# avi22bhattacharya/ThinkDiff-mlre

Measured on NVIDIA B200. Metric: aligner_train_tokens_per_sec, higher is better.
Workload: dtype bf16

## Files before the change

thinkdiff_mlre_b200/csrc/gemm_host.cuh:

```cuda
#pragma once
#include <cstdio>
#include <cstring>
#include <atomic>
#include <mutex>
#include <vector>

#include "gemm_sm100.cuh"

namespace td {

inline char* last_error_buf() {
  static thread_local char buf[512] = "";
  return buf;
}
#define TD_FAIL(code, ...)                                        \
  do {                                                            \
    snprintf(td::last_error_buf(), 512, __VA_ARGS__);             \
    return (code);                                                \
  } while (0)
#define TD_CUDA(expr)                                                                             \
  do {                                                                                            \
    cudaError_t _e = (expr);                                                                      \
    if (_e != cudaSuccess) TD_FAIL(-100 - int(_e), "%s failed: %s", #expr, cudaGetErrorString(_e)); \
  } while (0)
// ... 140 lines not shown
                            bool mn_major, int box_rows) {
  if (!mn_major)
    return encode_2d(map, CU_TENSOR_MAP_DATA_TYPE_BFLOAT16, ptr, (cuuint64_t)K, (cuuint64_t)rows, (cuuint64_t)ld * 2, kBlockK,
                     (cuuint32_t)box_rows, CU_TENSOR_MAP_SWIZZLE_128B, CU_TENSOR_MAP_L2_PROMOTION_L2_256B);
  return encode_2d(map, CU_TENSOR_MAP_DATA_TYPE_BFLOAT16, ptr, (cuuint64_t)rows, (cuuint64_t)K, (cuuint64_t)ld * 2, 64, kBlockK,
                   CU_TENSOR_MAP_SWIZZLE_128B, CU_TENSOR_MAP_L2_PROMOTION_L2_256B);
}
inline int make_epilogue_map(CUtensorMap* map, const void* ptr, long long rows, long long cols, long long ld, bool f32) {
  if (f32)
    return encode_2d(map, CU_TENSOR_MAP_DATA_TYPE_FLOAT32, ptr, (cuuint64_t)cols, (cuuint64_t)rows, (cuuint64_t)ld * 4, 32, 32,
                     CU_TENSOR_MAP_SWIZZLE_128B, CU_TENSOR_MAP_L2_PROMOTION_NONE);
  return encode_2d(map, CU_TENSOR_MAP_DATA_TYPE_BFLOAT16, ptr, (cuuint64_t)cols, (cuuint64_t)rows, (cuuint64_t)ld * 2, 32, 32,
                   CU_TENSOR_MAP_SWIZZLE_64B, CU_TENSOR_MAP_L2_PROMOTION_NONE);
}

struct GemmOperand {
  const void* ptr;
  long long ld;
  bool mn_major;
};

inline size_t gemm_sk_workspace_bytes() { return sizeof(float) * (size_t)device_sm_count() * kSkSlotFloats; }

inline void plan_schedule(GemmParams& p, int max_workers, bool stream_k) {
  const int tiles = p.num_m_blocks * p.num_n_blocks;
  const int KB = p.num_k_blocks;
  int W = max_workers;
  if (tiles < W) {
    long long by_k = (long long)tiles * KB / kMinTailKBlocks;
    long long w = stream_k ? (by_k > tiles ? by_k : tiles) : tiles;
    W = int(w < max_workers ? w : max_workers);
    if (W < 1) W = 1;
  }
  p.workers = W;
  p.full_waves = tiles / W;
  const int R = tiles - p.full_waves * W;
  p.tail_workers = 0; p.tail_q = 0; p.tail_r = 0;
  if (stream_k && R > 0) {
    const long long units = (long long)R * KB;
    long long wt = units / kMinTailKBlocks;
    if (wt < R) wt = R;
    if (wt > W) wt = W;
    p.tail_workers = int(wt);
    p.tail_q = int(units / wt);
    p.tail_r = int(units % wt);
  }
}

template <int CTAS, bool A_MN, bool B_MN, int EPI>
int launch_gemm(GemmOperand a, GemmOperand b, GemmParams p, void* ws, cudaStream_t stream, const char* tag = "gemm") {
  using S = GemmSmem<CTAS, EPI>;
  if (p.M <= 0 || p.N <= 0) return TD_OK;
  if (p.N % 32) TD_FAIL(TD_ERR_UNSUPPORTED, "GEMM N=%d must be a multiple of 32", p.N);
  if (p.K <= 0) TD_FAIL(TD_ERR_ARG, "GEMM K=%d must be positive (caller zero-fills empty contractions)", p.K);
  CUtensorMap ma, mb, mo0, mo1, maux;
  ScatterMaps smaps;
  memset(&mo0, 0, sizeof(mo0)); memset(&mo1, 0, sizeof(mo1)); memset(&maux, 0, sizeof(maux)); memset(&smaps, 0, sizeof(smaps));
  int rc = make_operand_map(&ma, a.ptr, p.M, p.K, a.ld, A_MN, kBlockM);
  if (rc) return rc;
  rc = make_operand_map(&mb, b.ptr, p.N, p.K, b.ld, B_MN, kBlockN / CTAS);
  if (rc) return rc;
  if (EPI != EPI_F32_SCATTER && p.out0 != nullptr) {
    rc = make_epilogue_map(&mo0, p.out0, p.M, p.N, p.ld_out, EPI == EPI_F32);
    if (rc) return rc;
  }
  if (EPI == EPI_BIAS_GELU) {
    rc = make_epilogue_map(&mo1, p.out1, p.M, p.N, p.ld_out, false);
    if (rc) return rc;
// ... 17 lines not shown
  p.sk_partials = static_cast<float*>(ws);
  p.sched_counter = next_sched_counter();
  if (!p.sched_counter) TD_FAIL(TD_ERR_DRIVER, "cannot allocate the tile-scheduler counters");
  p.sk_flags = nullptr;
  if (p.tail_workers > 0) {
    p.sk_flags = next_sk_flags();
    if (!p.sk_flags) TD_FAIL(TD_ERR_DRIVER, "cannot allocate the stream-K flag pool");
  }

  auto kern = gemm_bf16_kernel<CTAS, A_MN, B_MN, EPI>;
  static std::atomic<bool> attr_set[kMaxDevices];
  const int dev = current_device();
  if (dev < 0 || dev >= kMaxDevices) TD_FAIL(TD_ERR_DRIVER, "no current CUDA device");
  if (!attr_set[dev].load(std::memory_order_acquire)) {
    TD_CUDA(cudaFuncSetAttribute(kern, cudaFuncAttributeMaxDynamicSharedMemorySize, S::kTotal));
    attr_set[dev].store(true, std::memory_order_release);
  }
  cudaLaunchConfig_t cfg;
  memset(&cfg, 0, sizeof(cfg));
  cfg.gridDim = dim3(p.workers * CTAS);
  cfg.blockDim = dim3(kGemmThreads);
  cfg.dynamicSmemBytes = S::kTotal;
  cfg.stream = stream;
  cudaLaunchAttribute attr[1];
  attr[0].id = cudaLaunchAttributeClusterDimension;
  attr[0].val.clusterDim.x = CTAS;
  attr[0].val.clusterDim.y = 1;
  attr[0].val.clusterDim.z = 1;
  cfg.attrs = attr;
  cfg.numAttrs = 1;
  ProfScope prof(tag, 2.0 * double(p.M) * double(p.N) * double(p.K), stream);
  TD_CUDA(cudaLaunchKernelEx(&cfg, kern, ma, mb, mo0, mo1, maux, smaps, p));
  return TD_OK;
}

}
```

thinkdiff_mlre_b200/csrc/gemm_sm100.cuh:

```cuda
#pragma once
#include "ptx_sm100.cuh"

namespace td {

enum EpiKind : int {
  EPI_BF16 = 0,
  EPI_BIAS_GELU = 1,
  EPI_BIAS_SSQ = 2,
  EPI_DGELU = 3,
  EPI_F32 = 4,
  EPI_F32_SCATTER = 5,
};
constexpr int kMaxPeers = 8;

struct GemmParams {
  int M, N, K;
  int num_m_blocks, num_n_blocks, num_k_blocks;
  int workers;
  int full_waves;
  int tail_workers;
  int tail_q, tail_r;
  float* sk_partials;
  int* sk_flags;
  int* sched_counter;
// ... 11 lines not shown
  int scatter_rows;
  int raster_group_m;
  int raster_rot_m;
  int* post_signal[kMaxPeers];
  int post_signal_n;
};
struct ScatterMaps {
  CUtensorMap m[kMaxPeers];
};

constexpr int kBlockM = 128;
constexpr int kBlockN = 256;
constexpr int kBlockK = 64;
constexpr int kUmmaK = 16;
constexpr int kGemmThreads = 320;
#ifndef TD_ROLES_HI
#define TD_ROLES_HI 1
#endif
constexpr int kEpiWarp0 = TD_ROLES_HI ? 0 : 2;
constexpr int kProducerWarp = TD_ROLES_HI ? 8 : 0;
constexpr int kMmaWarp = TD_ROLES_HI ? 9 : 1;
constexpr int kAccStages = 2;
constexpr int kMinTailKBlocks = 8;

constexpr int kEpiWarps = 8;
constexpr int kEpiColsPerWarp = kBlockN / (kEpiWarps / 4);
constexpr int kEpiChunks = kEpiColsPerWarp / 32;
constexpr int kSkSlotFloats = kEpiWarps * kEpiChunks * 32 * 32;

#ifndef TD_MAX_STAGES
#define TD_MAX_STAGES 7
#endif

template <int EPI> struct EpiStage { static constexpr int kBytesPerWarp = 4096; };
template <> struct EpiStage<EPI_DGELU> { static constexpr int kBytesPerWarp = 6144; };
template <> struct EpiStage<EPI_F32> { static constexpr int kBytesPerWarp = 8192; };
template <> struct EpiStage<EPI_F32_SCATTER> { static constexpr int kBytesPerWarp = 8192; };

template <int EPI> struct StageCap { static constexpr int kMax = TD_MAX_STAGES; };
#ifndef TD_NO_CORESIDENCY
template <> struct StageCap<EPI_BIAS_GELU> { static constexpr int kMax = 5; };
template <> struct StageCap<EPI_F32> { static constexpr int kMax = 5; };
template <> struct StageCap<EPI_F32_SCATTER> { static constexpr int kMax = 5; };
#endif

template <int CTAS, int EPI>
// ... 348 lines not shown
    if constexpr (EPI == EPI_DGELU) tma_prefetch_desc(&tmap_aux);
    for (int s = 0; s < kStages; ++s) {
      mbar_init(&full_bar[s], 1);
      mbar_init(&empty_bar[s], 1);
    }
    for (int s = 0; s < kAccStages; ++s) {
      mbar_init(&acc_full_bar[s], 1);
      mbar_init(&acc_empty_bar[s], kEpiWarps * CTAS);
    }
    for (int s = 0; s < 2 * kEpiWarps; ++s) mbar_init(&aux_bar[s], 1);
    for (int s = 0; s < kSchedStages; ++s) {
      mbar_init(&sched_full_bar[s], 1);
      mbar_init(&sched_empty_bar[s], kSchedConsumers);
    }
    fence_mbar_init();
  }
  if (warp == kMmaWarp) {
    tmem_alloc<CTAS>(tmem_slot, 512);
    tmem_relinquish<CTAS>();
  }
  tc_fence_before();
  if constexpr (CTAS == 2) cluster_sync_all(); else __syncthreads();
  tc_fence_after();
  const uint32_t tmem_base = *tmem_slot;
  const int num_workers = gridDim.x / CTAS;
  const int n_units = num_units(p);

  auto sched_consume = [&](int ss, uint32_t sphase, bool whole_warp) -> int {
    mbar_wait_cluster(&sched_full_bar[ss], sphase);
    const int unit = *reinterpret_cast<volatile int*>(&sched_unit[ss]);
    if (whole_warp) __syncwarp();
    if (!whole_warp || lane == 0) {
      if constexpr (CTAS == 1) mbar_arrive(&sched_empty_bar[ss]);
      else mbar_arrive_cluster(&sched_empty_bar[ss], 0);
    }
    return unit;
  };

  if (warp == kProducerWarp) {
    if (lane == 0) {
      int stage = 0, ss = 0;
      uint32_t phase = 0, sphase = 0;
      int claimed = leader ? atomicAdd(p.sched_counter, 1) : 0;
      while (true) {
        int unit;
        if (leader) {
// ... 27 lines not shown
              if constexpr (CTAS == 1) tma_load_2d(sa, &tmap_a, &full_bar[stage], k0, a_row0);
              else tma_load_2d_pair(sa, &tmap_a, &full_bar[stage], k0, a_row0);
            } else {
#pragma unroll
              for (int j = 0; j < kBlockM / 64; ++j) {
                if constexpr (CTAS == 1) tma_load_2d(sa + j * (kBlockK * 128), &tmap_a, &full_bar[stage], a_row0 + j * 64, k0);
                else tma_load_2d_pair(sa + j * (kBlockK * 128), &tmap_a, &full_bar[stage], a_row0 + j * 64, k0);
              }
            }
            if constexpr (!B_MN) {
              if constexpr (CTAS == 1) tma_load_2d(sb, &tmap_b, &full_bar[stage], k0, b_row0);
              else tma_load_2d_pair(sb, &tmap_b, &full_bar[stage], k0, b_row0);
            } else {
#pragma unroll
              for (int j = 0; j < kBRows / 64; ++j) {
                if constexpr (CTAS == 1) tma_load_2d(sb + j * (kBlockK * 128), &tmap_b, &full_bar[stage], b_row0 + j * 64, k0);
                else tma_load_2d_pair(sb + j * (kBlockK * 128), &tmap_b, &full_bar[stage], b_row0 + j * 64, k0);
              }
            }
            if (++stage == kStages) { stage = 0; phase ^= 1; }
          }
        });
      }
      if (leader) {
        __threadfence();
        if (atomicAdd(p.sched_counter + 1, 1) == num_workers - 1) {
          p.sched_counter[0] = 0;
          p.sched_counter[1] = 0;
          __threadfence();
        }
      }
    }
    __syncwarp();
  } else if (warp == kMmaWarp) {
    if (leader && lane == 0) {
      constexpr uint32_t idesc = make_idesc_bf16(kBlockM * CTAS, kBlockN, A_MN, B_MN);
      constexpr uint32_t a_lbo = A_MN ? kBlockK * 128 : 16, b_lbo = B_MN ? kBlockK * 128 : 16;
      constexpr uint32_t sbo = 1024;
      constexpr uint32_t a_kstep = A_MN ? kUmmaK * 128 : kUmmaK * 2;
      constexpr uint32_t b_kstep = B_MN ? kUmmaK * 128 : kUmmaK * 2;
      int stage = 0, acc = 0, ss = 0;
      uint32_t phase = 0, acc_phase = 0, sphase = 0;
      while (true) {
        const int unit = sched_consume(ss, sphase, false);
        if (++ss == kSchedStages) { ss = 0; sphase ^= 1; }
        if (unit < 0) break;
// ... 81 lines not shown
```

thinkdiff_mlre_b200/csrc/ptx_sm100.cuh:

```cuda
#pragma once
#include <cuda.h>
#include <cuda_bf16.h>
#include <cuda_runtime.h>
#include <stdint.h>

namespace td {

__device__ __forceinline__ uint32_t smem_u32(const void* p) {
  return static_cast<uint32_t>(__cvta_generic_to_shared(p));
}

__device__ __forceinline__ uint64_t global_timer_ns() {
  uint64_t t;
  asm volatile("mov.u64 %0, %%globaltimer;" : "=l"(t));
  return t;
}

__device__ __forceinline__ void mbar_init(uint64_t* bar, uint32_t count) {
  asm volatile("mbarrier.init.shared::cta.b64 [%0], %1;" ::"r"(smem_u32(bar)), "r"(count));
}
__device__ __forceinline__ void fence_mbar_init() {
  asm volatile("fence.mbarrier_init.release.cluster;" ::: "memory");
}
__device__ __forceinline__ void fence_proxy_async_smem() {
// ... 78 lines not shown
  int v;
  asm volatile("ld.acquire.gpu.global.s32 %0, [%1];" : "=r"(v) : "l"(p) : "memory");
  return v;
}
__device__ __forceinline__ int ld_relaxed_gpu(const int* p) {
  int v;
  asm volatile("ld.relaxed.gpu.global.s32 %0, [%1];" : "=r"(v) : "l"(p) : "memory");
  return v;
}
__device__ __forceinline__ void spin_until_set(const int* p) {
  if (ld_relaxed_gpu(p) == 0) {
    const uint64_t t0 = global_timer_ns();
    while (ld_relaxed_gpu(p) == 0) {
      __nanosleep(64);
      if (global_timer_ns() - t0 > TD_MBAR_TIMEOUT_NS) {
        printf("td: stream-K flag timeout block %d thread %d\n", blockIdx.x, threadIdx.x);
        __trap();
      }
    }
  }
  asm volatile("fence.acq_rel.gpu;" ::: "memory");
}

__device__ __forceinline__ uint32_t cluster_ctarank() {
  uint32_t r;
  asm volatile("mov.u32 %0, %%cluster_ctarank;" : "=r"(r));
  return r;
}
__device__ __forceinline__ void cluster_sync_all() {
  asm volatile("barrier.cluster.arrive.release.aligned;\n barrier.cluster.wait.acquire.aligned;" ::: "memory");
}

__device__ __forceinline__ void fence_tensormap_acquire(const CUtensorMap* m) {
  asm volatile("fence.proxy.tensormap::generic.acquire.sys [%0], 128;" ::"l"(m) : "memory");
}

__device__ __forceinline__ void tma_prefetch_desc(const CUtensorMap* m) {
  asm volatile("prefetch.tensormap [%0];" ::"l"(m) : "memory");
}
__device__ __forceinline__ void tma_load_2d(void* dst, const CUtensorMap* map, uint64_t* bar, int c0, int c1) {
  asm volatile(
      "cp.async.bulk.tensor.2d.shared::cluster.global.mbarrier::complete_tx::bytes [%0], [%1, {%3, %4}], [%2];" ::"r"(
          smem_u32(dst)),
      "l"(map), "r"(smem_u32(bar)), "r"(c0), "r"(c1)
      : "memory");
}
// ... 162 lines not shown
```

thinkdiff_mlre_b200/csrc/rowops_sm100.cuh:

```cuda
#pragma once
#include "ptx_sm100.cuh"

namespace td {

__device__ __forceinline__ uint4 ld_stream(const uint4* p) {
  uint4 r;
  asm("ld.global.nc.L1::no_allocate.v4.u32 {%0, %1, %2, %3}, [%4];"
      : "=r"(r.x), "=r"(r.y), "=r"(r.z), "=r"(r.w)
      : "l"(p));
  return r;
}
#ifndef TD_ST_VARIANT
#define TD_ST_VARIANT 0
#endif
__device__ __forceinline__ void st_stream(uint4* p, const uint4& v) {
#if TD_ST_VARIANT == 0
  asm volatile("st.global.L1::no_allocate.v4.u32 [%0], {%1, %2, %3, %4};" ::"l"(p), "r"(v.x), "r"(v.y), "r"(v.z),
               "r"(v.w)
               : "memory");
#elif TD_ST_VARIANT == 1
  *p = v;
#else
  __stcs(p, v);
#endif
// ... 5 lines not shown
               : "l"(p));
#pragma unroll
  for (int i = 0; i < 8; ++i) r[i] = __uint_as_float(u[i]);
}
__device__ __forceinline__ void st256_evict_first(float* p, const float (&r)[8]) {
  asm volatile("st.global.L1::no_allocate.L2::evict_first.v8.b32 [%0], {%1, %2, %3, %4, %5, %6, %7, %8};" ::"l"(p),
               "r"(__float_as_uint(r[0])), "r"(__float_as_uint(r[1])), "r"(__float_as_uint(r[2])), "r"(__float_as_uint(r[3])),
               "r"(__float_as_uint(r[4])), "r"(__float_as_uint(r[5])), "r"(__float_as_uint(r[6])), "r"(__float_as_uint(r[7]))
               : "memory");
}

__device__ __forceinline__ float warp_sum(float v) {
#pragma unroll
  for (int o = 16; o >= 1; o >>= 1) v += __shfl_xor_sync(0xffffffffu, v, o);
  return v;
}
__device__ __forceinline__ float warp_max(float v) {
#pragma unroll
  for (int o = 16; o >= 1; o >>= 1) v = fmaxf(v, __shfl_xor_sync(0xffffffffu, v, o));
  return v;
}

__global__ void cu_seqlens_kernel(const int* __restrict__ lens, int B, int* __restrict__ cu) {
  __shared__ int warp_tot[32];
  __shared__ int carry;
  if (threadIdx.x == 0) { carry = 0; cu[0] = 0; }
  __syncthreads();
  for (int base = 0; base < B; base += blockDim.x) {
    const int i = base + threadIdx.x;
    int v = i < B ? lens[i] : 0;
    const int lane = threadIdx.x & 31, w = threadIdx.x >> 5;
    int x = v;
#pragma unroll
    for (int o = 1; o < 32; o <<= 1) {
      int y = __shfl_up_sync(0xffffffffu, x, o);
      if (lane >= o) x += y;
    }
    if (lane == 31) warp_tot[w] = x;
    __syncthreads();
    if (w == 0) {
      int t = lane < (blockDim.x >> 5) ? warp_tot[lane] : 0;
#pragma unroll
      for (int o = 1; o < 32; o <<= 1) {
        int y = __shfl_up_sync(0xffffffffu, t, o);
        if (lane >= o) t += y;
      }
      warp_tot[lane] = t;
    }
    __syncthreads();
    const int before = carry + (w ? warp_tot[w - 1] : 0);
    if (i < B) cu[i + 1] = before + x;
    __syncthreads();
    if (threadIdx.x == 0) carry += warp_tot[(blockDim.x >> 5) - 1];
    __syncthreads();
  }
}

constexpr int kPackMaxStagedSeqs = 2048;

template <bool PADDED>
__global__ void __launch_bounds__(256)
pack_rows_kernel(const uint4* __restrict__ src, const long long* __restrict__ src_row_start,
                 const int* __restrict__ cu, int B, long long dst_rows, int Lmax, int vec_per_row,
                 uint4* __restrict__ dst, long long* __restrict__ mask, long long* __restrict__ src_row_out,
                 const uint4* __restrict__ src2 = nullptr) {
  __shared__ int s_cu[kPackMaxStagedSeqs + 1];
  __shared__ long long s_start[kPackMaxStagedSeqs];
  const bool staged = B <= kPackMaxStagedSeqs;
  if (staged) {
    for (int i = threadIdx.x; i <= B; i += blockDim.x) s_cu[i] = cu[i];
    for (int i = threadIdx.x; i < B; i += blockDim.x) s_start[i] = src_row_start[i];
    __syncthreads();
  }
  const int* cu_t = staged ? s_cu : cu;
  const long long* start_t = staged ? s_start : src_row_start;
  const int lane = threadIdx.x & 31;
  const long long warp0 = (long long)blockIdx.x * (blockDim.x >> 5) + (threadIdx.x >> 5);
  const long long nwarps = (long long)gridDim.x * (blockDim.x >> 5);
  for (long long r = warp0; r < dst_rows; r += nwarps) {
    int i, j;
    bool valid = true;
    if constexpr (PADDED) {
      i = int(r / Lmax);
      j = int(r - (long long)i * Lmax);
      valid = j < (cu_t[i + 1] - cu_t[i]);
      if (mask != nullptr && lane == 0) mask[r] = valid ? 1ll : 0ll;
    } else {
      int lo = 0, hi = B;
// ... 359 lines not shown
    float a = 0.f, b = 0.f;
    for (int i = 0; i < 8; ++i) { a += s_sq[i]; b += s_bad[i]; }
    if (b != 0.f) atomicAdd(stats, b);
    atomicAdd(stats + 1, a);
  }
}

constexpr int kNormMseMaxRows = 1024;

template <bool T_BF16>
struct NormMseRow {
  uint4 h;
  uint4 t0;
  uint4 t1;
};

template <bool T_BF16>
__global__ void __launch_bounds__(kNormBwdThreads, 1)
norm_mse_bwd_kernel(const __nv_bfloat16* __restrict__ h2, const float* __restrict__ ssq_part, int P, float eps,
                    const float* __restrict__ g, const void* __restrict__ t_in,
                    const long long* __restrict__ t_row_index, int M, int D, int rows_per_cta, float dy_coef,
                    __nv_bfloat16* __restrict__ dh2, float* __restrict__ dg_part, float* __restrict__ db2_part,
                    float* __restrict__ loss_part) {
  constexpr int R = kNormBwdRows;
  constexpr int PF = T_BF16 ? 2 : 1;
  constexpr int NB = PF + 1;
  constexpr int NW = kNormBwdThreads / 32;
  static_assert(NW == 16, "the partial-sum butterfly assumes 16 warps");
  __shared__ float red[2][R][NW];
  __shared__ float lred[NW];
  __shared__ float rs_sm[kNormMseMaxRows];
  __shared__ long long ti_sm[kNormMseMaxRows];
  const int t = threadIdx.x, lane = t & 31, w = t >> 5;
  const bool col_ok = t * 8 < D;
  const int row_begin = blockIdx.x * rows_per_cta;
  const int row_end = min(M, row_begin + rows_per_cta);
  float gg[8], adg[8], adb[8];
#pragma unroll
  for (int q = 0; q < 8; ++q) { gg[q] = col_ok ? g[t * 8 + q] : 0.f; adg[q] = 0.f; adb[q] = 0.f; }
  const float inv_d = 1.0f / float(D);
  float loss_acc = 0.f;

  for (int b0 = row_begin; b0 < row_end; b0 += kNormMseMaxRows) {
    const int b1 = min(row_end, b0 + kNormMseMaxRows);
    __syncthreads();
    for (int i = t; i < b1 - b0; i += kNormBwdThreads)
// ... 113 lines not shown
  if (lane == 0) lred[w] = loss_acc;
  __syncthreads();
  if (t == 0) {
    float tot_loss = 0.f;
    for (int i = 0; i < NW; ++i) tot_loss += lred[i];
    loss_part[blockIdx.x] = tot_loss;
  }
}

struct FinishJob { const float* part; float* out; int P; int use_scale_ptr; };
struct FinishParams {
  FinishJob job[3];
  int njobs, N;
  float scale;
  const float* scale_ptr;
  int accumulate;
  float* stats;
  const float* loss_part; int loss_P; float* loss_out; float loss_div;
  float* post[8]; int n_post; const float* post_base; long long post_numel;
};

__global__ void __launch_bounds__(256)
finish_kernel(const FinishParams f) {
  __shared__ float red[8][33];
  const int lane = threadIdx.x & 31, w = threadIdx.x >> 5;
  if (int(blockIdx.y) == f.njobs) {
    if (blockIdx.x != 0 || f.loss_out == nullptr) return;
    float acc = 0.f;
    for (int i = threadIdx.x; i < f.loss_P; i += blockDim.x) acc += f.loss_part[i];
    acc = warp_sum(acc);
    if (lane == 0) red[w][0] = acc;
    __syncthreads();
    if (threadIdx.x == 0) {
      float tot = 0.f;
      for (int i = 0; i < 8; ++i) tot += red[i][0];
      f.loss_out[0] = tot / f.loss_div;
    }
    return;
  }
  const FinishJob j = f.job[blockIdx.y];
  const int col = blockIdx.x * 32 + lane;
  const int N = f.N, P = j.P;
  float a0 = 0.f, a1 = 0.f, a2 = 0.f, a3 = 0.f;
  if (col < N) {
    int p = w;
    for (; p + 24 < P; p += 32) {
// ... 129 lines not shown
        if constexpr (Y_BF16) {
          st_stream(reinterpret_cast<uint4*>(reinterpret_cast<__nv_bfloat16*>(dy_out) + (long long)row * D) + v,
                    make_uint4(pack_bf16x2(d[0], d[1]), pack_bf16x2(d[2], d[3]), pack_bf16x2(d[4], d[5]), pack_bf16x2(d[6], d[7])));
        } else {
          uint4* p = reinterpret_cast<uint4*>(reinterpret_cast<float*>(dy_out) + (long long)row * D) + 2 * v;
          st_stream(p, make_uint4(__float_as_uint(d[0]), __float_as_uint(d[1]), __float_as_uint(d[2]), __float_as_uint(d[3])));
          st_stream(p + 1, make_uint4(__float_as_uint(d[4]), __float_as_uint(d[5]), __float_as_uint(d[6]), __float_as_uint(d[7])));
        }
      }
    }
  }
  acc = warp_sum(acc);
  if (lane == 0) wsum[threadIdx.x >> 5] = acc;
  __syncthreads();
  if (threadIdx.x == 0) {
    float tot = 0.f;
    for (int i = 0; i < (blockDim.x >> 5); ++i) tot += wsum[i];
    loss_part[blockIdx.x] = tot;
  }
}

__global__ void loss_finish_kernel(const float* __restrict__ part, int P, const float* __restrict__ meta, float d_or_1,
                                   float* __restrict__ loss, float n_valid_if_no_meta = 0.f) {
  __shared__ float wsum[32];
  float acc = 0.f;
  for (int i = threadIdx.x; i < P; i += blockDim.x) acc += part[i];
  acc = warp_sum(acc);
  if ((threadIdx.x & 31) == 0) wsum[threadIdx.x >> 5] = acc;
  __syncthreads();
  if (threadIdx.x == 0) {
    float tot = 0.f;
    for (int i = 0; i < (blockDim.x >> 5); ++i) tot += wsum[i];
    loss[0] = tot / ((meta != nullptr ? meta[0] : n_valid_if_no_meta) * d_or_1);
  }
}

constexpr int kCeThreads = 256;

template <bool Z_BF16>
__global__ void __launch_bounds__(kCeThreads, 3)
masked_ce_kernel(const void* __restrict__ z_in, const long long* __restrict__ labels, int V, const float* __restrict__ meta,
                 float grad_scale, void* __restrict__ dz_out, float* __restrict__ row_loss) {
  extern __shared__ uint4 zs[];
  __shared__ float red_m[kCeThreads / 32], red_s[kCeThreads / 32];
  __shared__ float bc_m, bc_s;
  constexpr int EPV = Z_BF16 ? 8 : 4;
// ... 91 lines not shown
```

thinkdiff_mlre_b200/csrc/td_api.cu:

```cuda
#include "thinkdiff_b200.h"

#include "gemm_host.cuh"
#include "rowops_sm100.cuh"
#include "peer_sm100.cuh"
#include "attn_sm100.cuh"

#include <cmath>

using namespace td;

namespace {

inline size_t align_up(size_t x, size_t a) { return (x + a - 1) / a * a; }

struct Carver {
  uint8_t* base;
  size_t off = 0;
  explicit Carver(void* p) : base(static_cast<uint8_t*>(p)) {}
  template <class T>
  T* take(size_t n) {
    T* r = reinterpret_cast<T*>(base + off);
    off = align_up(off + n * sizeof(T), 256);
    return r;
  }
// ... 6 lines not shown
  return TD_OK;
}
#define TD_DEVICE_OR_RETURN()      \
  do {                             \
    int _rc = check_device();      \
    if (_rc) return _rc;           \
  } while (0)

template <class K>
inline void prefer_max_shared(K kernel) {
  static std::atomic<bool> done[kMaxDevices];
  const int dev = current_device();
  if (dev < 0 || dev >= kMaxDevices || done[dev].load(std::memory_order_acquire)) return;
  cudaFuncSetAttribute(kernel, cudaFuncAttributePreferredSharedMemoryCarveout, cudaSharedmemCarveoutMaxShared);
  cudaGetLastError();
  done[dev].store(true, std::memory_order_release);
}

inline int grid_for_rows(long long rows, int rows_per_block, int blocks_per_sm) {
  const long long want = (rows + rows_per_block - 1) / rows_per_block;
  const long long cap = (long long)device_sm_count() * blocks_per_sm;
  return int(want < cap ? (want > 0 ? want : 1) : cap);
}

inline int norm_bwd_grid(long long M, int* rows_per_cta) {
  int ctas = device_sm_count() * 2;
  long long rpc = (M + ctas - 1) / ctas;
  rpc = (rpc + kNormBwdRows - 1) / kNormBwdRows * kNormBwdRows;
  if (rpc < kNormBwdRows) rpc = kNormBwdRows;
  *rows_per_cta = int(rpc);
  return int((M + rpc - 1) / rpc);
}

inline int norm_mse_grid(long long M, int* rows_per_cta) {
  int ctas = device_sm_count();
  long long rpc = (M + ctas - 1) / ctas;
  rpc = (rpc + kNormBwdRows - 1) / kNormBwdRows * kNormBwdRows;
  if (rpc < kNormBwdRows) rpc = kNormBwdRows;
  *rows_per_cta = int(rpc);
  return int((M + rpc - 1) / rpc);
}

inline bool dims_ok(int Din, int D) { return Din > 0 && D > 0 && Din % 64 == 0 && D % 64 == 0 && D <= 8 * kNormBwdThreads; }

}

// ... 38 lines not shown

int32_t td_profile_timeline(char* buf, int32_t buflen) {
  Profiler& p = Profiler::get();
  std::lock_guard<std::mutex> lock(p.mu);
  int off = 0;
  if (buflen > 0) buf[0] = 0;
  if (p.recs.empty()) return TD_OK;
  cudaEvent_t base = p.recs[0].e0;
  for (auto& r : p.recs) {
    if (cudaEventSynchronize(r.e1) != cudaSuccess) TD_FAIL(TD_ERR_DRIVER, "td_profile_timeline: event sync failed");
    float t0 = 0.f, t1 = 0.f;
    cudaEventElapsedTime(&t0, base, r.e0);
    cudaEventElapsedTime(&t1, base, r.e1);
    int w = snprintf(buf + off, buflen > off ? buflen - off : 0, "%s,%p,%.4f,%.4f\n", r.tag, (void*)r.stream, t0, t1);
    if (w < 0 || off + w >= buflen) TD_FAIL(TD_ERR_ARG, "td_profile_timeline: buffer too small");
    off += w;
  }
  return TD_OK;
}

int32_t td_cu_seqlens(const int32_t* lens, int32_t B, int32_t* cu, td_stream_t stream) {
  TD_DEVICE_OR_RETURN();
  if (B < 0 || !cu || (B > 0 && !lens)) TD_FAIL(TD_ERR_ARG, "td_cu_seqlens: bad arguments");
  cu_seqlens_kernel<<<1, 1024, 0, (cudaStream_t)stream>>>(lens, B, cu);
  TD_CUDA(cudaGetLastError());
  return TD_OK;
}

int32_t td_pack_varlen_indexed(const void* src, const int64_t* src_row_start, const int32_t* cu, int32_t B,
                               int64_t total_rows, int64_t row_bytes, void* dst, int64_t* src_row_out, td_stream_t stream);

int32_t td_pack_varlen(const void* src, const int64_t* src_row_start, const int32_t* cu, int32_t B, int64_t total_rows,
                       int64_t row_bytes, void* dst, td_stream_t stream) {
  return td_pack_varlen_indexed(src, src_row_start, cu, B, total_rows, row_bytes, dst, nullptr, stream);
}

int32_t td_pack_varlen_indexed(const void* src, const int64_t* src_row_start, const int32_t* cu, int32_t B,
                               int64_t total_rows, int64_t row_bytes, void* dst, int64_t* src_row_out, td_stream_t stream) {
  TD_DEVICE_OR_RETURN();
  if (B < 0 || total_rows < 0 || row_bytes <= 0 || row_bytes % 16)
    TD_FAIL(TD_ERR_ARG, "td_pack_varlen: row_bytes=%lld must be a positive multiple of 16", (long long)row_bytes);
  if (total_rows == 0 || B == 0) return TD_OK;
  if (!src || !src_row_start || !cu || !dst) TD_FAIL(TD_ERR_ARG, "td_pack_varlen: null pointer");
  if ((reinterpret_cast<uintptr_t>(src) | reinterpret_cast<uintptr_t>(dst)) & 15)
    TD_FAIL(TD_ERR_ARG, "td_pack_varlen: buffers must be 16-byte aligned");
  const int grid = grid_for_rows(total_rows, 8, 8);
  {
    ProfScope prof("pack_varlen", 2.0 * double(total_rows) * double(row_bytes), (cudaStream_t)stream);
    pack_rows_kernel<false><<<grid, 256, 0, (cudaStream_t)stream>>>(
        static_cast<const uint4*>(src), reinterpret_cast<const long long*>(src_row_start), cu, B, total_rows, 0,
        int(row_bytes / 16), static_cast<uint4*>(dst), nullptr, reinterpret_cast<long long*>(src_row_out));
  }
  TD_CUDA(cudaGetLastError());
  return TD_OK;
}

int32_t td_pack_varlen2(const void* src, const void* src2, const int64_t* src_row_start, const int32_t* cu, int32_t B,
                        int64_t total_rows, int64_t row_bytes, void* dst, td_stream_t stream) {
  TD_DEVICE_OR_RETURN();
  if (B < 0 || total_rows < 0 || row_bytes <= 0 || row_bytes % 16)
    TD_FAIL(TD_ERR_ARG, "td_pack_varlen2: row_bytes=%lld must be a positive multiple of 16", (long long)row_bytes);
  if (total_rows == 0 || B == 0) return TD_OK;
  if (!src || !src2 || !src_row_start || !cu || !dst) TD_FAIL(TD_ERR_ARG, "td_pack_varlen2: null pointer");
  if ((reinterpret_cast<uintptr_t>(src) | reinterpret_cast<uintptr_t>(src2) | reinterpret_cast<uintptr_t>(dst)) & 15)
    TD_FAIL(TD_ERR_ARG, "td_pack_varlen2: buffers must be 16-byte aligned");
  const int grid = grid_for_rows(total_rows, 8, 8);
  {
    ProfScope prof("pack_varlen", 2.0 * double(total_rows) * double(row_bytes), (cudaStream_t)stream);
    pack_rows_kernel<false><<<grid, 256, 0, (cudaStream_t)stream>>>(
        static_cast<const uint4*>(src), reinterpret_cast<const long long*>(src_row_start), cu, B, total_rows, 0,
        int(row_bytes / 16), static_cast<uint4*>(dst), nullptr, nullptr, static_cast<const uint4*>(src2));
  }
  TD_CUDA(cudaGetLastError());
  return TD_OK;
}

int32_t td_pack_padded(const void* src, const int64_t* src_row_start, const int32_t* cu, int32_t B, int32_t L_max,
                       int64_t row_bytes, void* dst, int64_t* mask, td_stream_t stream) {
  TD_DEVICE_OR_RETURN();
  if (B < 0 || L_max < 0 || row_bytes <= 0 || row_bytes % 16)
    TD_FAIL(TD_ERR_ARG, "td_pack_padded: row_bytes=%lld must be a positive multiple of 16", (long long)row_bytes);
  if (B == 0 || L_max == 0) return TD_OK;
  if (!src_row_start || !cu || !dst) TD_FAIL(TD_ERR_ARG, "td_pack_padded: null pointer");
  if ((reinterpret_cast<uintptr_t>(src) | reinterpret_cast<uintptr_t>(dst)) & 15)
    TD_FAIL(TD_ERR_ARG, "td_pack_padded: buffers must be 16-byte aligned");
  const long long rows = (long long)B * L_max;
  const int grid = grid_for_rows(rows, 8, 8);
  {
    ProfScope prof("pack_padded", 2.0 * double(rows) * double(row_bytes), (cudaStream_t)stream);
    pack_rows_kernel<true><<<grid, 256, 0, (cudaStream_t)stream>>>(
        static_cast<const uint4*>(src), reinterpret_cast<const long long*>(src_row_start), cu, B, rows, L_max,
        int(row_bytes / 16), static_cast<uint4*>(dst), reinterpret_cast<long long*>(mask), nullptr);
  }
  TD_CUDA(cudaGetLastError());
  return TD_OK;
}

int32_t td_cast_f32_to_bf16(const float* src, void* dst, int64_t n, td_stream_t stream) {
  TD_DEVICE_OR_RETURN();
  if (n < 0) TD_FAIL(TD_ERR_ARG, "td_cast_f32_to_bf16: n < 0");
  if (n == 0) return TD_OK;
  if ((reinterpret_cast<uintptr_t>(src) | reinterpret_cast<uintptr_t>(dst)) & 15)
    TD_FAIL(TD_ERR_ARG, "td_cast_f32_to_bf16: buffers must be 16-byte aligned");
  const int grid = grid_for_rows((n + 7) / 8, 256, 8);
  {
    ProfScope prof("cast_f32_to_bf16", 6.0 * double(n), (cudaStream_t)stream);
    cast_f32_to_bf16_kernel<<<grid, 256, 0, (cudaStream_t)stream>>>(src, static_cast<__nv_bfloat16*>(dst), n);
  }
  TD_CUDA(cudaGetLastError());
  return TD_OK;
}

int32_t td_rmsnorm_fwd(const void* x, const float* g, float eps, int64_t M, int32_t D, void* y, int32_t y_dtype,
                       float* rstd, td_stream_t stream) {
  TD_DEVICE_OR_RETURN();
  if (M < 0 || D <= 0 || D % 8 || D > 8 * 32 * kNormFwdMaxVec)
    TD_FAIL(TD_ERR_ARG, "td_rmsnorm_fwd: D=%d must be a positive multiple of 8, at most %d", D, 8 * 32 * kNormFwdMaxVec);
// ... 272 lines not shown
    if (rc) return rc;
  }
  if (do_gelu || do_small2 || ex.loss_out != nullptr) {
    FinishParams f;
    memset(&f, 0, sizeof(f));
    f.N = D; f.scale = scale; f.accumulate = ex.accumulate; f.stats = ex.stats;
    f.scale_ptr = scale_ptr;
    if (do_small2) {
      f.job[f.njobs++] = FinishJob{ex.np->dg_part, dg, ex.np->grid, 1};
      f.job[f.njobs++] = FinishJob{ex.np->db_part, db2, ex.np->grid, 1};
    }
    if (do_gelu) {
      const int slabs = int((M + 2 * kBlockM - 1) / (2 * kBlockM)) * 2 * 4;
      f.job[f.njobs++] = FinishJob{w.db1_part, db1, slabs, 0};
    }
    if (ex.loss_out != nullptr && ex.np != nullptr) {
      f.loss_part = ex.np->loss_part; f.loss_P = ex.np->grid; f.loss_out = ex.loss_out; f.loss_div = ex.loss_div;
    }
    if (sc != nullptr && sc->n_post > 0) {
      for (int o = 0; o < sc->n_post; ++o) f.post[o] = sc->post[o];
      f.n_post = sc->n_post; f.post_base = sc->post_base; f.post_numel = sc->post_numel;
    }
    if (f.njobs > 0 || f.loss_out != nullptr) {
      finish_kernel<<<dim3((D + 31) / 32, f.njobs + (f.loss_out ? 1 : 0)), 256, 0, st>>>(f);
      TD_CUDA(cudaGetLastError());
    }
  }
  if (phases & (TD_BWD_PHASE_GELU_W1 | TD_BWD_PHASE_W1_ONLY)) {
    memset(&p, 0, sizeof(p));
    p.M = D; p.N = Din; p.K = int(M); p.ld_out = Din; p.alpha = scale; p.out0 = dW1; p.stats = ex.stats; p.accumulate = ex.accumulate;
    const bool last = !(phases & (TD_BWD_PHASE_NORM_W2 | TD_BWD_PHASE_W2_ONLY));
    int rc = launch_dw_gemm({w.dh0, D, true}, {x, Din, true}, p, sc ? sc->dW1 : nullptr, world, sc ? sc->rank : -1, w.sk, st,
                            world ? "gemm_dW1_scatter" : "gemm_dW1", last ? sc : nullptr);
    if (rc) return rc;
  }
  if (phases & (TD_BWD_PHASE_NORM_W2 | TD_BWD_PHASE_W2_ONLY)) {
    memset(&p, 0, sizeof(p));
    p.M = D; p.N = D; p.K = int(M); p.ld_out = D; p.alpha = scale; p.alpha_ptr = scale_ptr; p.out0 = dW2; p.stats = ex.stats;
    p.accumulate = ex.accumulate;
    int rc = launch_dw_gemm({dh2, D, true}, {h1, D, true}, p, sc ? sc->dW2 : nullptr, world, sc ? sc->rank : -1, w.sk, st,
                            world ? "gemm_dW2_scatter" : "gemm_dW2", sc);
    if (rc) return rc;
  }
  return TD_OK;
}

int zero_grads(int32_t Din, int32_t D, float* dW1, float* db1, float* dW2, float* db2, float* dg, int32_t phases,
               cudaStream_t st) {
// ... 62 lines not shown
  const int nparts = (D + kEpiColsPerWarp - 1) / kEpiColsPerWarp;
  __nv_bfloat16* h2 = c.take<__nv_bfloat16>((size_t)M * D);
  NormPartials np = carve_norm_partials(norm_partials, M, D);

  GemmParams p;
  int rc;
  if (stages & TD_FWD_STAGE_LINEAR1) {
    memset(&p, 0, sizeof(p));
    p.M = int(M); p.N = D; p.K = Din; p.ld_out = D; p.alpha = 1.f;
    p.out0 = h0; p.out1 = h1; p.bias = static_cast<const __nv_bfloat16*>(b1);
    rc = launch_gemm<2, false, false, EPI_BIAS_GELU>({x, Din, false}, {W1, Din, false}, p, w.sk, st, "gemm_fwd1_bias_gelu");
    if (rc) return rc;
  }
  if (!(stages & TD_FWD_STAGE_REST)) return TD_OK;
  memset(&p, 0, sizeof(p));
  p.M = int(M); p.N = D; p.K = D; p.ld_out = D; p.alpha = 1.f;
  p.out0 = h2; p.bias = static_cast<const __nv_bfloat16*>(b2); p.red0 = w.ssq_part;
  rc = launch_gemm<2, false, false, EPI_BIAS_SSQ>({h1, D, false}, {W2, D, false}, p, w.sk, st, "gemm_fwd2_bias_ssq");
  if (rc) return rc;
  const float dy_coef = 2.0f / (float(M) * float(D));
  const long long* tri = reinterpret_cast<const long long*>(target_row_index);
  {
    ProfScope prof("norm_mse_bwd_fused", double(M) * D * (4.0 + (target_dtype == TD_DTYPE_BF16 ? 2.0 : 4.0)), st);
    if (target_dtype == TD_DTYPE_BF16)
      norm_mse_bwd_kernel<true><<<np.grid, kNormBwdThreads, 0, st>>>(h2, w.ssq_part, nparts, eps, g, target, tri, int(M), D, np.rows_per_cta,
                                                                     dy_coef, static_cast<__nv_bfloat16*>(dh2), np.dg_part, np.db_part, np.loss_part);
    else
      norm_mse_bwd_kernel<false><<<np.grid, kNormBwdThreads, 0, st>>>(h2, w.ssq_part, nparts, eps, g, target, tri, int(M), D, np.rows_per_cta,
                                                                      dy_coef, static_cast<__nv_bfloat16*>(dh2), np.dg_part, np.db_part, np.loss_part);
  }
  TD_CUDA(cudaGetLastError());
  if (!(stages & TD_FWD_STAGE_DEFER_LOSS)) {
    loss_finish_kernel<<<1, 256, 0, st>>>(np.loss_part, np.grid, nullptr, float(D), loss, float(M));
    TD_CUDA(cudaGetLastError());
  }
  return TD_OK;
}

}
namespace {
int bwd_dh2_impl(const void* dh2, const void* x, const void* h0, const void* h1, const void* W2,
                 const void* norm_partials, int64_t M, int32_t Din, int32_t D,
                 float grad_scale, const float* grad_scale_ptr, float* dW1, float* db1, float* dW2, float* db2,
                 float* dg, float* loss_out, float* stats, int32_t accumulate, void* ws, int64_t ws_bytes, int32_t phases,
                 td_stream_t stream, const ScatterDst* sc) {
  TD_DEVICE_OR_RETURN();
  if (!dims_ok(Din, D)) TD_FAIL(TD_ERR_UNSUPPORTED, "td_aligner_bwd_dh2: Din=%d, D=%d must be multiples of 64 (D <= 4096)", Din, D);
  if (M <= 0 || M > 0x7fffffffll / D) TD_FAIL(TD_ERR_ARG, "td_aligner_bwd_dh2: M=%lld out of range", (long long)M);
  if (ws_bytes < td_aligner_bwd_workspace_bytes(M, Din, D)) TD_FAIL(TD_ERR_ARG, "td_aligner_bwd_dh2: workspace too small");
  if (accumulate && sc) TD_FAIL(TD_ERR_UNSUPPORTED, "td_aligner_bwd_dh2_scatter: gradient accumulation needs local outputs");
  cudaStream_t st = (cudaStream_t)stream;
  BwdWorkspace w = carve_bwd(ws, M, D);
  if ((phases & (TD_BWD_PHASE_NORM_W2 | TD_BWD_PHASE_W2_ONLY)) && (!dh2 || !h1 || !dW2))
    TD_FAIL(TD_ERR_ARG, "td_aligner_bwd_dh2: null pointer (dW2)");
  NormPartials np;
  BwdExtras ex;
  ex.stats = stats; ex.accumulate = accumulate;
// ... 597 lines not shown
```

Baseline: 6.848 million.

## Enable programmatic dependent launch across kernels and cost-tune stream-K tail split

Launches the GEMM and row-op kernels with programmatic stream serialization. Each kernel calls griddepcontrol.wait before touching dependent data and launch_dependents early, so a kernel's prologue (barrier init, TMEM alloc) can overlap the tail of the previous kernel. The stream-K tail planner now searches worker counts and models fold cost from how many workers share a tile, and shrinks the grid when there are no full waves. The intent is to cut launch gaps and tail imbalance, at the cost of PDL ordering subtleties and extra host-side planning work.

```diff
diff --git a/thinkdiff_mlre_b200/csrc/gemm_host.cuh b/thinkdiff_mlre_b200/csrc/gemm_host.cuh
--- a/thinkdiff_mlre_b200/csrc/gemm_host.cuh
+++ b/thinkdiff_mlre_b200/csrc/gemm_host.cuh
@@ -186,6 +186,16 @@
 
 inline size_t gemm_sk_workspace_bytes() { return sizeof(float) * (size_t)device_sm_count() * kSkSlotFloats; }
 
+inline int max_tail_participants(const GemmParams& p, int R) {
+  const int KB = p.num_k_blocks;
+  int most = 1;
+  for (int t = 0; t < R; ++t) {
+    const int n = sk_worker_of(p, (t + 1) * KB - 1) - sk_worker_of(p, t * KB) + 1;
+    if (n > most) most = n;
+  }
+  return most;
+}
+
 inline void plan_schedule(GemmParams& p, int max_workers, bool stream_k) {
   const int tiles = p.num_m_blocks * p.num_n_blocks;
   const int KB = p.num_k_blocks;
@@ -202,12 +212,21 @@
   p.tail_workers = 0; p.tail_q = 0; p.tail_r = 0;
   if (stream_k && R > 0) {
     const long long units = (long long)R * KB;
-    long long wt = units / kMinTailKBlocks;
-    if (wt < R) wt = R;
-    if (wt > W) wt = W;
-    p.tail_workers = int(wt);
-    p.tail_q = int(units / wt);
-    p.tail_r = int(units % wt);
+    long long hi = units / kMinTailKBlocks;
+    if (hi < R) hi = R;
+    if (hi > W) hi = W;
+    long long best_cost = -1;
+    int best = int(hi);
+    for (int wt = int(hi); wt >= R; --wt) {
+      p.tail_q = int(units / wt);
+      p.tail_r = int(units % wt);
+      const long long cost = (units + wt - 1) / wt + (long long)kTailFoldKBlocks * (max_tail_participants(p, R) - 1);
+      if (best_cost < 0 || cost < best_cost) { best_cost = cost; best = wt; }
+    }
+    p.tail_workers = best;
+    p.tail_q = int(units / best);
+    p.tail_r = int(units % best);
+    if (p.full_waves == 0) p.workers = best;
   }
 }
 
@@ -271,13 +290,15 @@
   cfg.blockDim = dim3(kGemmThreads);
   cfg.dynamicSmemBytes = S::kTotal;
   cfg.stream = stream;
-  cudaLaunchAttribute attr[1];
+  cudaLaunchAttribute attr[2];
   attr[0].id = cudaLaunchAttributeClusterDimension;
   attr[0].val.clusterDim.x = CTAS;
   attr[0].val.clusterDim.y = 1;
   attr[0].val.clusterDim.z = 1;
+  attr[1].id = cudaLaunchAttributeProgrammaticStreamSerialization;
+  attr[1].val.programmaticStreamSerializationAllowed = 1;
   cfg.attrs = attr;
-  cfg.numAttrs = 1;
+  cfg.numAttrs = 2;
   ProfScope prof(tag, 2.0 * double(p.M) * double(p.N) * double(p.K), stream);
   TD_CUDA(cudaLaunchKernelEx(&cfg, kern, ma, mb, mo0, mo1, maux, smaps, p));
   return TD_OK;
diff --git a/thinkdiff_mlre_b200/csrc/gemm_sm100.cuh b/thinkdiff_mlre_b200/csrc/gemm_sm100.cuh
--- a/thinkdiff_mlre_b200/csrc/gemm_sm100.cuh
+++ b/thinkdiff_mlre_b200/csrc/gemm_sm100.cuh
@@ -57,6 +57,10 @@
 constexpr int kMmaWarp = TD_ROLES_HI ? 9 : 1;
 constexpr int kAccStages = 2;
 constexpr int kMinTailKBlocks = 8;
+#ifndef TD_SK_FOLD_KBLOCKS
+#define TD_SK_FOLD_KBLOCKS 8
+#endif
+constexpr int kTailFoldKBlocks = TD_SK_FOLD_KBLOCKS;
 
 constexpr int kEpiWarps = 8;
 constexpr int kEpiColsPerWarp = kBlockN / (kEpiWarps / 4);
@@ -451,6 +455,7 @@
   tc_fence_before();
   if constexpr (CTAS == 2) cluster_sync_all(); else __syncthreads();
   tc_fence_after();
+  grid_dependency_wait();
   const uint32_t tmem_base = *tmem_slot;
   const int num_workers = gridDim.x / CTAS;
   const int n_units = num_units(p);
@@ -524,6 +529,7 @@
           }
         });
       }
+      grid_launch_dependents();
       if (leader) {
         __threadfence();
         if (atomicAdd(p.sched_counter + 1, 1) == num_workers - 1) {
diff --git a/thinkdiff_mlre_b200/csrc/ptx_sm100.cuh b/thinkdiff_mlre_b200/csrc/ptx_sm100.cuh
--- a/thinkdiff_mlre_b200/csrc/ptx_sm100.cuh
+++ b/thinkdiff_mlre_b200/csrc/ptx_sm100.cuh
@@ -124,6 +124,9 @@
   asm volatile("fence.acq_rel.gpu;" ::: "memory");
 }
 
+__device__ __forceinline__ void grid_dependency_wait() { asm volatile("griddepcontrol.wait;" ::: "memory"); }
+__device__ __forceinline__ void grid_launch_dependents() { asm volatile("griddepcontrol.launch_dependents;" ::: "memory"); }
+
 __device__ __forceinline__ uint32_t cluster_ctarank() {
   uint32_t r;
   asm volatile("mov.u32 %0, %%cluster_ctarank;" : "=r"(r));
diff --git a/thinkdiff_mlre_b200/csrc/rowops_sm100.cuh b/thinkdiff_mlre_b200/csrc/rowops_sm100.cuh
--- a/thinkdiff_mlre_b200/csrc/rowops_sm100.cuh
+++ b/thinkdiff_mlre_b200/csrc/rowops_sm100.cuh
@@ -51,6 +51,8 @@
 }
 
 __global__ void cu_seqlens_kernel(const int* __restrict__ lens, int B, int* __restrict__ cu) {
+  grid_dependency_wait();
+  grid_launch_dependents();
   __shared__ int warp_tot[32];
   __shared__ int carry;
   if (threadIdx.x == 0) { carry = 0; cu[0] = 0; }
@@ -93,6 +95,8 @@
                  const int* __restrict__ cu, int B, long long dst_rows, int Lmax, int vec_per_row,
                  uint4* __restrict__ dst, long long* __restrict__ mask, long long* __restrict__ src_row_out,
                  const uint4* __restrict__ src2 = nullptr) {
+  grid_dependency_wait();
+  grid_launch_dependents();
   __shared__ int s_cu[kPackMaxStagedSeqs + 1];
   __shared__ long long s_start[kPackMaxStagedSeqs];
   const bool staged = B <= kPackMaxStagedSeqs;
@@ -498,6 +502,8 @@
                     const long long* __restrict__ t_row_index, int M, int D, int rows_per_cta, float dy_coef,
                     __nv_bfloat16* __restrict__ dh2, float* __restrict__ dg_part, float* __restrict__ db2_part,
                     float* __restrict__ loss_part) {
+  grid_dependency_wait();
+  grid_launch_dependents();
   constexpr int R = kNormBwdRows;
   constexpr int PF = T_BF16 ? 2 : 1;
   constexpr int NB = PF + 1;
@@ -657,6 +663,8 @@
 
 __global__ void __launch_bounds__(256)
 finish_kernel(const FinishParams f) {
+  grid_dependency_wait();
+  grid_launch_dependents();
   __shared__ float red[8][33];
   const int lane = threadIdx.x & 31, w = threadIdx.x >> 5;
   if (int(blockIdx.y) == f.njobs) {
@@ -832,6 +840,8 @@
 
 __global__ void loss_finish_kernel(const float* __restrict__ part, int P, const float* __restrict__ meta, float d_or_1,
                                    float* __restrict__ loss, float n_valid_if_no_meta = 0.f) {
+  grid_dependency_wait();
+  grid_launch_dependents();
   __shared__ float wsum[32];
   float acc = 0.f;
   for (int i = threadIdx.x; i < P; i += blockDim.x) acc += part[i];
diff --git a/thinkdiff_mlre_b200/csrc/td_api.cu b/thinkdiff_mlre_b200/csrc/td_api.cu
--- a/thinkdiff_mlre_b200/csrc/td_api.cu
+++ b/thinkdiff_mlre_b200/csrc/td_api.cu
@@ -52,6 +52,22 @@
   const long long cap = (long long)device_sm_count() * blocks_per_sm;
   return int(want < cap ? (want > 0 ? want : 1) : cap);
 }
+
+struct PdlConfig {
+  cudaLaunchAttribute attr;
+  cudaLaunchConfig_t cfg;
+  PdlConfig(dim3 grid, dim3 block, cudaStream_t st) {
+    memset(&cfg, 0, sizeof(cfg));
+    cfg.gridDim = grid;
+    cfg.blockDim = block;
+    cfg.stream = st;
+    attr.id = cudaLaunchAttributeProgrammaticStreamSerialization;
+    attr.val.programmaticStreamSerializationAllowed = 1;
+    cfg.attrs = &attr;
+    cfg.numAttrs = 1;
+  }
+  PdlConfig(const PdlConfig&) = delete;
+};
 
 inline int norm_bwd_grid(long long M, int* rows_per_cta) {
   int ctas = device_sm_count() * 2;
@@ -136,8 +152,8 @@
 int32_t td_cu_seqlens(const int32_t* lens, int32_t B, int32_t* cu, td_stream_t stream) {
   TD_DEVICE_OR_RETURN();
   if (B < 0 || !cu || (B > 0 && !lens)) TD_FAIL(TD_ERR_ARG, "td_cu_seqlens: bad arguments");
-  cu_seqlens_kernel<<<1, 1024, 0, (cudaStream_t)stream>>>(lens, B, cu);
-  TD_CUDA(cudaGetLastError());
+  PdlConfig l(1, 1024, (cudaStream_t)stream);
+  TD_CUDA(cudaLaunchKernelEx(&l.cfg, cu_seqlens_kernel, lens, B, cu));
   return TD_OK;
 }
 
@@ -161,11 +177,11 @@
   const int grid = grid_for_rows(total_rows, 8, 8);
   {
     ProfScope prof("pack_varlen", 2.0 * double(total_rows) * double(row_bytes), (cudaStream_t)stream);
-    pack_rows_kernel<false><<<grid, 256, 0, (cudaStream_t)stream>>>(
-        static_cast<const uint4*>(src), reinterpret_cast<const long long*>(src_row_start), cu, B, total_rows, 0,
-        int(row_bytes / 16), static_cast<uint4*>(dst), nullptr, reinterpret_cast<long long*>(src_row_out));
-  }
-  TD_CUDA(cudaGetLastError());
+    PdlConfig l(grid, 256, (cudaStream_t)stream);
+    TD_CUDA(cudaLaunchKernelEx(&l.cfg, pack_rows_kernel<false>, static_cast<const uint4*>(src),
+                               reinterpret_cast<const long long*>(src_row_start), cu, B, total_rows, 0, int(row_bytes / 16),
+                               static_cast<uint4*>(dst), nullptr, reinterpret_cast<long long*>(src_row_out), nullptr));
+  }
   return TD_OK;
 }
 
@@ -181,11 +197,11 @@
   const int grid = grid_for_rows(total_rows, 8, 8);
   {
     ProfScope prof("pack_varlen", 2.0 * double(total_rows) * double(row_bytes), (cudaStream_t)stream);
-    pack_rows_kernel<false><<<grid, 256, 0, (cudaStream_t)stream>>>(
-        static_cast<const uint4*>(src), reinterpret_cast<const long long*>(src_row_start), cu, B, total_rows, 0,
-        int(row_bytes / 16), static_cast<uint4*>(dst), nullptr, nullptr, static_cast<const uint4*>(src2));
-  }
-  TD_CUDA(cudaGetLastError());
+    PdlConfig l(grid, 256, (cudaStream_t)stream);
+    TD_CUDA(cudaLaunchKernelEx(&l.cfg, pack_rows_kernel<false>, static_cast<const uint4*>(src),
+                               reinterpret_cast<const long long*>(src_row_start), cu, B, total_rows, 0, int(row_bytes / 16),
+                               static_cast<uint4*>(dst), nullptr, nullptr, static_cast<const uint4*>(src2)));
+  }
   return TD_OK;
 }
 
@@ -202,11 +218,11 @@
   const int grid = grid_for_rows(rows, 8, 8);
   {
     ProfScope prof("pack_padded", 2.0 * double(rows) * double(row_bytes), (cudaStream_t)stream);
-    pack_rows_kernel<true><<<grid, 256, 0, (cudaStream_t)stream>>>(
-        static_cast<const uint4*>(src), reinterpret_cast<const long long*>(src_row_start), cu, B, rows, L_max,
-        int(row_bytes / 16), static_cast<uint4*>(dst), reinterpret_cast<long long*>(mask), nullptr);
-  }
-  TD_CUDA(cudaGetLastError());
+    PdlConfig l(grid, 256, (cudaStream_t)stream);
+    TD_CUDA(cudaLaunchKernelEx(&l.cfg, pack_rows_kernel<true>, static_cast<const uint4*>(src),
+                               reinterpret_cast<const long long*>(src_row_start), cu, B, rows, L_max, int(row_bytes / 16),
+                               static_cast<uint4*>(dst), reinterpret_cast<long long*>(mask), nullptr, nullptr));
+  }
   return TD_OK;
 }
 
@@ -525,8 +541,8 @@
       f.n_post = sc->n_post; f.post_base = sc->post_base; f.post_numel = sc->post_numel;
     }
     if (f.njobs > 0 || f.loss_out != nullptr) {
-      finish_kernel<<<dim3((D + 31) / 32, f.njobs + (f.loss_out ? 1 : 0)), 256, 0, st>>>(f);
-      TD_CUDA(cudaGetLastError());
+      PdlConfig l(dim3((D + 31) / 32, f.njobs + (f.loss_out ? 1 : 0)), 256, st);
+      TD_CUDA(cudaLaunchKernelEx(&l.cfg, finish_kernel, f));
     }
   }
   if (phases & (TD_BWD_PHASE_GELU_W1 | TD_BWD_PHASE_W1_ONLY)) {
@@ -635,17 +651,15 @@
   const long long* tri = reinterpret_cast<const long long*>(target_row_index);
   {
     ProfScope prof("norm_mse_bwd_fused", double(M) * D * (4.0 + (target_dtype == TD_DTYPE_BF16 ? 2.0 : 4.0)), st);
-    if (target_dtype == TD_DTYPE_BF16)
-      norm_mse_bwd_kernel<true><<<np.grid, kNormBwdThreads, 0, st>>>(h2, w.ssq_part, nparts, eps, g, target, tri, int(M), D, np.rows_per_cta,
-                                                                     dy_coef, static_cast<__nv_bfloat16*>(dh2), np.dg_part, np.db_part, np.loss_part);
-    else
-      norm_mse_bwd_kernel<false><<<np.grid, kNormBwdThreads, 0, st>>>(h2, w.ssq_part, nparts, eps, g, target, tri, int(M), D, np.rows_per_cta,
-                                                                      dy_coef, static_cast<__nv_bfloat16*>(dh2), np.dg_part, np.db_part, np.loss_part);
-  }
-  TD_CUDA(cudaGetLastError());
+    PdlConfig l(np.grid, kNormBwdThreads, st);
+    TD_CUDA(cudaLaunchKernelEx(&l.cfg, target_dtype == TD_DTYPE_BF16 ? norm_mse_bwd_kernel<true> : norm_mse_bwd_kernel<false>, h2,
+                               w.ssq_part, nparts, eps, g, target, tri, int(M), D, np.rows_per_cta, dy_coef,
+                               static_cast<__nv_bfloat16*>(dh2), np.dg_part, np.db_part, np.loss_part));
+  }
   if (!(stages & TD_FWD_STAGE_DEFER_LOSS)) {
-    loss_finish_kernel<<<1, 256, 0, st>>>(np.loss_part, np.grid, nullptr, float(D), loss, float(M));
-    TD_CUDA(cudaGetLastError());
+    PdlConfig l(1, 256, st);
+    TD_CUDA(cudaLaunchKernelEx(&l.cfg, loss_finish_kernel, static_cast<const float*>(np.loss_part), np.grid,
+                               static_cast<const float*>(nullptr), float(D), loss, float(M)));
   }
   return TD_OK;
 }
```

Result: faster. 7.081 million (median of 6 runs) (+3.4%).
